# clovaai/frostnet

Hardware: AMD Instinct MI355X
Metric: images/sec FrostNet-Large 224x224 QAT fwd+bwd (higher is better)
Workload: dtype int8; 1 GPU; FrostNet-Large int8 fake-quant QAT fwd+bwd + GradBoost-SGD step (noise on; StatAssist FP epoch is a one-off before it), batch=512/GPU, 224x224 NHWC, qnnpack qconfig v0 (per-tensor); per_gpu_batch=512, global_batch=512, resolution=224, parallelism=dp1, hip_graph=True, grad_dtype=bf16

## Files before the change

frostnet_amd/_lib.py:

```python
import ctypes as C
import os

import torch

_HERE = os.path.dirname(os.path.abspath(__file__))
LIB_PATH = os.environ.get("FROST_HIP_LIB", os.path.join(_HERE, "libfrost_hip.so"))
_lib = None

P, I, L, F, D = C.c_void_p, C.c_int, C.c_int64, C.c_float, C.c_double

Q_MIN, Q_MAX, Q_SCALE, Q_ZP, Q_FQMIN, Q_FQMAX, Q_INV, Q_QMAX, Q_OBS_EN, Q_FQ_EN, Q_STRIDE = 0, 1, 2, 3, 4, 5, 6, 7, 8, 10, 12
COEF_ROWS = int(os.environ.get("FROST_COEF_ROWS_ALLOC", "14"))
COEF_ROWS_NAMED = 8
DWQ_NC, DWQ_SPREAD_MAX = int(os.environ.get("FROST_DWQ_NC", "4")), 32768
COEF_A, COEF_B = 0, 1
COEF_M, COEF_R, COEF_K1, COEF_S1, COEF_S2, COEF_VFRAC = 2, 3, 4, 5, 6, 7
STATS_BYTES_PER_CH = 24 * int(os.environ.get("FROST_STATS_TABLES", "4"))


class FrostWDesc(C.Structure):
    _fields_ = [("w", P), ("gamma", P), ("rvar", P), ("qrec", P), ("wq_pack", P), ("wsum", P), ("minmax2", P),
                ("wt_pack", P), ("wscale", P), ("wmin", P), ("wmax", P), ("cout", C.c_int32), ("cin_g", C.c_int32), ("kk", C.c_int32), ("kind", C.c_int32),
                ("cpad", C.c_int32), ("kpad", C.c_int32), ("reserved0", C.c_int32), ("reserved1", C.c_int32)]

# ... 125 lines not shown
    "frost_dw_conv_fwd_fin": [P, P, P, P, I, I, I, I, I, I, P, P, P],
    "frost_dw_conv_fwd": [P, P, P, P, I, I, I, I, I, I, I, P, P, P, I, P, P],
    "frost_stem_im2col": [P, P, I, I, I, P, P],
    "frost_stem_wgrad_remap": [P, I, I, P, P],
    "frost_conv_finalize": [P, L, I, P, P, P, P, P, P, P, I, I, I, P, P, P, P],
    "frost_cat_observe": [P, P, P, I, P],
    "frost_cat_requant": [P, P, I, P, P, I, L, P, P, P],
    "frost_add_minmax": [P, P, P, P, L, P, P],
    "frost_add_minmax_observe": [P, P, P, P, L, P, P, I, P],
    "frost_add_requant": [P, P, P, P, L, P, P, P],
    "frost_avgpool": [P, P, I, I, I, P, P, P],
    "frost_classifier_fwd": [P, P, P, P, I, I, I, P, P, P],
    "frost_pw_conv_bwd": [P, P, P, P, P, P, L, I, I, I, P, P, I, P, P, P, I, P],
    "frost_pw_wgrad": [P, P, P, L, I, I, P, P],
    "frost_pw_bwd_fused_ok": [L, I, I],
    "frost_pw_conv_int": [P, P, P, P, L, I, I, P, P],
    "frost_pw_ew": [P, L, I, P, P, I, I, P, P, P],
    "frost_pw_ew_emit_add": [P, L, I, P, P, I, P, P, P, P, P, I, P],
    "frost_pw_ew_add_bwd": [P, L, I, P, P, I, I, P, P, P, P, P, P, I, P, P],
    "frost_pw_conv_fwd_keep": [P, P, P, P, L, I, I, P, P, P, P],
    "frost_pwc_bwd_ok": [L, I, I],
    "frost_pwc_conv_bwd": [P, P, P, P, L, I, I, I, P, P, I, P, P, P],
    "frost_pwc_conv_fwd_emit": [P, P, P, P, L, I, I, P, P, P, P],
    "frost_block_supported": [I, I, I, I, I, I],
    "frost_block_fwd": [P, P],
    "frost_block_bwd": [P, P, P],
    "frost_block_expand_dw_stats": [P, P, P, P, P, P, P, I, I, I, I, I, P, P, I, P, P, P],
    "frost_block_dw_stats": [P, P, P, P, I, I, I, I, I, P, P, P],
    "frost_block_dw_reduce_supported": [I, I, I, I, I, I],
    "frost_block_dw_bwd_supported": [I, I, I, I, I],
    "frost_block_dw_bwd_reduce": [P, P, P, P, I, I, I, I, I, P, P, I, P, P],
    "frost_block_dw_bwd": [P, P, P, P, P, P, I, I, I, I, I, P, P, I, P, P, P, P],
    "frost_block_dw_bwd_c1": [P, P, P, P, P, P, I, I, I, I, I, P, P, I, P, P, P, P, P, P, P, P, I, I, P],
    "frost_block_dw_bwd_c1_ok": [I, I, I, I, I, I],
    "frost_block_dw_reduce": [P, P, P, P, P, P, I, P, I, I, I, I, I, P, P, I, P, P, P, P],
    "frost_pw_dgrad_wide_ok": [L, I, I],
    "frost_pw_dgrad_wide": [P, P, P, L, I, I, P, I, P],
    "frost_pw_conv_bwd_fused": [P, P, P, P, P, P, L, I, I, P, P, I, P, P, P, I, P, P],
    "frost_dw_conv_bwd": [P, P, P, P, P, I, I, I, I, I, I, I, P, P, I, P, P, P],
    "frost_dw_conv_bwd_dc_wgrad": [P, P, P, P, P, I, I, I, I, I, I, P, P, I, P, P, P, P],
    "frost_dw_dgrad": [P, P, P, I, I, I, I, I, I, P, I, P, P],
    "frost_dw_wgrad": [P, P, P, I, I, I, I, I, I, P, P],
    "frost_dw_bwd_fused_ok": [I, I, I, I, I],
    "frost_dw_bwd_fused": [P, P, P, P, P, P, I, I, I, I, I, I, P, P, I, P, P, P, P],
    "frost_dw_bwd_fused_c1_ok": [I, I, I, I, I, I],
    "frost_dw_bwd_fused_c1": [P, P, P, P, P, P, I, I, I, I, I, I, P, P, I, P, P, P, P, P, P, P, P, I, I, P],
# ... 196 lines not shown
```

frostnet_amd/csrc/frost_block.hip:

```cpp
#include "frost_common.h"

typedef int v2i __attribute__((ext_vector_type(2)));
#include <stdlib.h>

__device__ __forceinline__ int blk_xcd_item(int b, int total, int on) {
  if (!on || b >= (total & ~31)) return b;
  const int xcd = b & 7, j = b >> 3;
  return (j >> 2) * 32 + xcd * 4 + (j & 3);
}
__device__ __forceinline__ int blk_xcd_run(int b, int total, int run) {
  if (run < 2 || b >= total - total % (8 * run)) return b;
  const int xcd = b & 7, j = b >> 3;
  return (j / run) * (8 * run) + xcd * run + (j % run);
}
static int blk_xcd_on() { static const int on = getenv("FROST_BLK_XCD") ? atoi(getenv("FROST_BLK_XCD")) : 1; return on; }

struct BlkAP {
  const int8_t* x; const float* qx;
  const int8_t* w1; const int32_t* wsum1;
  const float* coef1; const float* qy1; int8_t* y1;
  const int8_t* wq2; const int32_t* wsum2;
  uint8_t* stats2; FrostFinDesc fin;
  int n, cin, c, cpad, KS, kstr, nchunk, csplit, imgs, rounds, xrun;
};
// ... 1459 lines not shown
  int cpw = cpw_env > 0 ? cpw_env : 2;
  if (cpw > p.nchunk) cpw = p.nchunk;
  p.csplit = (p.nchunk + cpw - 1) / cpw;
  static const int rounds_env = getenv("FROST_BLK_ROUNDS_A") ? atoi(getenv("FROST_BLK_ROUNDS_A")) : 0;
  p.imgs = imgs_env > 0 ? imgs_env : 0;
  p.rounds = rounds_env > 0 ? rounds_env : (h == 14 ? 2 : 1);
  hipStream_t s = as_stream(stream);
#define BLK_A(KK, HH, NWW, KSS) if (k == KK && h == HH && p.KS == KSS) return launch_blk_a<KK, HH, NWW, KSS>(p, s);
  BLK_A(3, 7, 4, 2) BLK_A(3, 7, 4, 3) BLK_A(3, 7, 4, 4) BLK_A(3, 7, 4, 5) BLK_A(5, 7, 4, 2) BLK_A(5, 7, 4, 3) BLK_A(5, 7, 4, 4) BLK_A(5, 7, 4, 5)
  BLK_A(3, 14, 8, 1) BLK_A(3, 14, 8, 2) BLK_A(3, 14, 8, 3) BLK_A(5, 14, 8, 1) BLK_A(5, 14, 8, 2) BLK_A(5, 14, 8, 3)
#undef BLK_A
  FROST_REQUIRE(false, "block_expand_dw: no instance");
  return 1;
}

extern "C" int frost_pw_conv_fwd_fin(const int8_t*, const float*, const int8_t*, const int32_t*, int64_t, int, int, void*, const FrostFinDesc*, void*);
extern "C" int frost_pw_ew(const int32_t*, int64_t, int, float*, const float*, int, int, const uint16_t*, void*, void*);
extern "C" int frost_pw_dgrad_wide(const uint16_t*, const uint16_t*, const float*, int64_t, int, int, uint16_t*, int, void*);
extern "C" int frost_pw_wgrad(const uint16_t*, const int8_t*, const float*, int64_t, int, int, float*, void*);
extern "C" int frost_pw_conv_bwd(const int8_t*, const float*, const int8_t*, const int32_t*, const uint16_t*, const float*, int64_t, int, int, int, float*, const float*, int,
                                 const uint16_t*, uint16_t*, uint16_t*, int, void*);
extern "C" int frost_pwc_bwd_ok(int64_t, int, int);
extern "C" int frost_pwc_conv_bwd(const int8_t*, const float*, const int8_t*, const int32_t*, int64_t, int, int, int, float*, const float*, int, const uint16_t*, uint16_t*, void*);

static int blk_desc_check(const FrostBlockDesc* d) {
  FROST_REQUIRE(d && d->x && d->y1 && d->y2 && d->y3 && d->conv_out3, "block: incomplete descriptor");
  FROST_REQUIRE(d->conv2.cout == d->conv1.cout && d->conv1.k == 1 && d->reduce.k == 1, "block: conv1 / reduce_conv are 1x1, conv2 is depthwise over conv1's channels");
  FROST_REQUIRE(frost_block_supported(d->h, d->w, d->conv2.k, 1, d->cin, d->conv1.cout) && frost_block_dw_reduce_supported(d->h, d->w, d->conv2.k, 1, d->conv1.cout, d->reduce.cout)
                && d->reduce.cout < d->conv1.cout, "block: unsupported shape (14x14 / 7x7 maps, depthwise stride 1, reduce_conv narrower than the expanded tensor)");
  return 0;
}

extern "C" int frost_block_fwd(const FrostBlockDesc* d, void* stream) {
  if (int rc = blk_desc_check(d)) return rc;
  const int64_t npix = (int64_t)d->n * d->h * d->w;
  const FrostBlockLayer &l1 = d->conv1, &l2 = d->conv2, &l3 = d->reduce;
  int rc = frost_pw_conv_fwd_fin(d->x, d->qrec_x, l1.wq_pack, l1.wsum, npix, d->cin, l1.cout, l1.stats, &l1.fin, stream);
  if (rc) return rc;
  rc = frost_block_expand_dw_stats(d->x, d->qrec_x, l1.wq_pack, l1.wsum, l1.fin.coef, l1.fin.qrec_y, d->y1, d->n, d->h, d->w, d->cin, l1.cout, l2.wq_pack, l2.wsum, l2.k, l2.stats,
                                   &l2.fin, stream);
  if (rc) return rc;
  rc = frost_block_dw_reduce(d->y1, l1.fin.qrec_y, l2.wq_pack, l2.wsum, l2.fin.coef, l2.fin.qrec_y, l2.fin.relu, d->y2, d->n, d->h, d->w, l1.cout, l2.k, l3.wq_pack, l3.wsum, l3.cout,
                             d->conv_out3, l3.stats, &l3.fin, stream);
  if (rc) return rc;
  return frost_pw_ew(d->conv_out3, npix, l3.cout, l3.fin.coef, l3.fin.qrec_y, l3.fin.relu, 2, nullptr, d->y3, stream);
}

extern "C" int frost_block_bwd(const FrostBlockDesc* d, const FrostBlockBwd* b, void* stream) {
  if (int rc = blk_desc_check(d)) return rc;
  FROST_REQUIRE(b && b->gout3 && b->dc3 && b->g2 && b->g1 && b->dc1, "block_bwd: incomplete gradient buffers");
  const int64_t npix = (int64_t)d->n * d->h * d->w;
  const FrostBlockLayer &l1 = d->conv1, &l2 = d->conv2, &l3 = d->reduce;
  hipStream_t ms = as_stream(stream), ss = b->side_stream ? as_stream(b->side_stream) : ms;
  hipEvent_t ev = nullptr;
  auto fork = [&]() { if (ss != ms) { if (!ev) hipEventCreateWithFlags(&ev, hipEventDisableTiming); hipEventRecord(ev, ms); hipStreamWaitEvent(ss, ev, 0); } };
  int rc;
  if ((rc = frost_pw_ew(d->conv_out3, npix, l3.cout, l3.fin.coef, l3.fin.qrec_y, l3.fin.relu, 0, b->gout3, nullptr, stream))) return rc;
  if ((rc = frost_pw_ew(d->conv_out3, npix, l3.cout, l3.fin.coef, l3.fin.qrec_y, l3.fin.relu, 1, b->gout3, b->dc3, stream))) return rc;
  fork();
  if ((rc = frost_pw_dgrad_wide(b->dc3, l3.wt_pack, l3.fin.qrec_w, npix, l1.cout, l3.cout, b->g2, 0, stream))) return rc;
  if ((rc = frost_pw_wgrad(b->dc3, d->y2, l2.fin.qrec_y, npix, l1.cout, l3.cout, l3.dwq, (void*)ss))) return rc;
  if ((rc = frost_block_dw_bwd_reduce(d->y1, l1.fin.qrec_y, l2.wq_pack, l2.wsum, d->n, d->h, d->w, l1.cout, l2.k, l2.fin.coef, l2.fin.qrec_y, l2.fin.relu, b->g2, stream))) return rc;
  if ((rc = frost_block_dw_bwd(d->y1, l1.fin.qrec_y, l2.wq_pack, l2.wsum, l2.fin.qrec_w, l2.fin.wscale, d->n, d->h, d->w, l1.cout, l2.k, l2.fin.coef, l2.fin.qrec_y, l2.fin.relu,
                               b->g2, b->g1, l2.dwq, stream))) return rc;
  const bool pwc = frost_pwc_bwd_ok(npix, d->cin, l1.cout) != 0;
  if (pwc && npix <= 131072) rc = frost_pwc_conv_bwd(d->x, d->qrec_x, l1.wq_pack, l1.wsum, npix, d->cin, l1.cout, 0, l1.fin.coef, l1.fin.qrec_y, l1.fin.relu, b->g1, nullptr, stream);
  else rc = frost_pw_conv_bwd(d->x, d->qrec_x, l1.wq_pack, l1.wsum, l1.wt_pack, l1.fin.qrec_w, npix, d->cin, l1.cout, 0, l1.fin.coef, l1.fin.qrec_y, l1.fin.relu, b->g1, nullptr, nullptr, 0, stream);
  if (rc) return rc;
  if (pwc) rc = frost_pwc_conv_bwd(d->x, d->qrec_x, l1.wq_pack, l1.wsum, npix, d->cin, l1.cout, 1, l1.fin.coef, l1.fin.qrec_y, l1.fin.relu, b->g1, b->dc1, stream);
  else rc = frost_pw_conv_bwd(d->x, d->qrec_x, l1.wq_pack, l1.wsum, l1.wt_pack, l1.fin.qrec_w, npix, d->cin, l1.cout, 1, l1.fin.coef, l1.fin.qrec_y, l1.fin.relu, b->g1, b->dc1, nullptr, 0, stream);
  if (rc) return rc;
  fork();
  if (b->dx && (rc = frost_pw_dgrad_wide(b->dc1, l1.wt_pack, l1.fin.qrec_w, npix, d->cin, l1.cout, b->dx, 0, stream))) return rc;
  if ((rc = frost_pw_wgrad(b->dc1, d->x, d->qrec_x, npix, d->cin, l1.cout, l1.dwq, (void*)ss))) return rc;
  if (ss != ms) {
    hipEventRecord(ev, ss); hipStreamWaitEvent(ms, ev, 0);
  }
  if (ev) hipEventDestroy(ev);
  return frost_check_launch("block_bwd");
}

struct SqCatP {
  const int8_t* x; const float* qx; const int8_t* w; const int32_t* wsum; const float* coef; const float* qsq; const float* qcat;
  int8_t* ysq; int8_t* ycat; int64_t npix; int cin, r, cpad, kstr;
  int cvt;
};
template <int KSM>
__global__ __launch_bounds__(256) void k_sq_emit_cat(const SqCatP p) {
  extern __shared__ __attribute__((aligned(16))) uint8_t smem[];
  uint8_t* const xs = smem;
  uint8_t* const lut = smem + 128 * p.kstr;
  const int tid = threadIdx.x, lane = tid & 63, wv = __builtin_amdgcn_readfirstlane(tid >> 6);
  const int j = lane & 15, g = lane >> 4;
  const int64_t p0 = (int64_t)blockIdx.x * 128;
  {
    const QP A = load_qp(p.qsq), B = load_qp(p.qx), Y = load_qp(p.qcat);
// ... 495 lines not shown
```

frostnet_amd/csrc/frost_pwc.hip:

```cpp
#include "frost_common.h"

struct PwcP {
  const int8_t* x; const float* qx; const int8_t* w; const int32_t* wsum;
  float* coef; const float* qy; const uint16_t* gout; uint16_t* dc; int8_t* y;
  int64_t npix; int cin, c, cpad, kstr, nchunk, csplit, relu, sr; float inv_count;
  uint8_t* stats; FrostFinDesc fin; unsigned fin_total; int ptpw; int64_t ntiles;
};

__device__ __forceinline__ void pwc_barrier() { asm volatile("s_waitcnt lgkmcnt(0)\n\ts_barrier" ::: "memory"); }
template <int CTRL>
__device__ __forceinline__ float pwc_dpp_add(float v) { return v + __int_as_float(__builtin_amdgcn_update_dpp(0, __float_as_int(v), CTRL, 0xf, 0xf, false)); }
__device__ __forceinline__ float pwc_row_sum(float v) { v = pwc_dpp_add<0x111>(v); v = pwc_dpp_add<0x112>(v); v = pwc_dpp_add<0x114>(v); v = pwc_dpp_add<0x118>(v); return v; }

#define PWC_PX 64
template <int MODE, int KSM>
__global__ __launch_bounds__(256, 4) void k_pwc(const PwcP p) {
  extern __shared__ __attribute__((aligned(16))) uint8_t smem[];
  uint8_t* const xs = smem;
  uint8_t* const gwin = smem + PWC_PX * p.kstr;
  const int tid = threadIdx.x, lane = tid & 63, w = __builtin_amdgcn_readfirstlane(tid >> 6);
  const int j = lane & 15, g = lane >> 4;
  const int cs = (int)blockIdx.x % p.csplit; const int64_t tile = (int64_t)blockIdx.x / p.csplit;
  const int chunk_lo = (cs * p.nchunk) / p.csplit, chunk_hi = ((cs + 1) * p.nchunk) / p.csplit;
  const int cw = (chunk_hi - chunk_lo) * 64;
// ... 179 lines not shown

extern "C" int frost_pwc_conv_bwd(const int8_t* x, const float* qrec_x, const int8_t* wq_pack, const int32_t* wsum, int64_t npix, int cin, int cout, int pass,
                                  float* coef, const float* qrec_y, int relu, const uint16_t* gout, uint16_t* dc, void* stream) {
  FROST_REQUIRE(frost_pwc_bwd_ok(npix, cin, cout) && (pass == 0 || (pass == 1 && dc)), "pwc_conv_bwd: unsupported layer or pass");
  PwcP p = {};
  p.x = x; p.qx = qrec_x; p.w = wq_pack; p.wsum = wsum; p.coef = coef; p.qy = qrec_y; p.gout = gout; p.dc = dc; p.npix = npix; p.cin = cin; p.c = cout;
  p.cpad = round_up(cout, 16); const int KS = (cin + 63) / 64; p.kstr = KS * 64 + 16; p.nchunk = (cout + 63) / 64; p.relu = relu; p.sr = frost_sr_enabled();
  p.inv_count = 1.0f / (float)npix;
  static const int cpw_env = getenv("FROST_PWC_CPW") ? atoi(getenv("FROST_PWC_CPW")) : 0;
  const int64_t tiles = (npix + PWC_PX - 1) / PWC_PX;
  int cpw = cpw_env > 0 ? cpw_env : (int)((tiles * p.nchunk + 2047) / 2048);
  if (cpw < 2) cpw = 2;
  if (cpw > p.nchunk) cpw = p.nchunk;
  if (cpw > 12) cpw = 12;
  p.csplit = (p.nchunk + cpw - 1) / cpw;
  hipStream_t s = as_stream(stream);
#define PWC_GO(KK) if (KS == KK) return pass == 0 ? launch_pwc<0, KK>(p, s) : launch_pwc<1, KK>(p, s);
  PWC_GO(1) PWC_GO(2) PWC_GO(3) PWC_GO(4) PWC_GO(5)
#undef PWC_GO
  FROST_REQUIRE(false, "pwc_conv_bwd: no instance");
  return 1;
}

extern "C" int frost_pwc_conv_fwd_emit(const int8_t* x, const float* qrec_x, const int8_t* wq_pack, const int32_t* wsum, int64_t npix, int cin, int cout,
                                       const float* coef, const float* qrec_y, int8_t* y, void* stream) {
  FROST_REQUIRE(frost_pwc_bwd_ok(npix, cin, cout) && y, "pwc_conv_fwd_emit: unsupported layer");
  PwcP p = {};
  p.x = x; p.qx = qrec_x; p.w = wq_pack; p.wsum = wsum; p.coef = (float*)coef; p.qy = qrec_y; p.y = y; p.npix = npix; p.cin = cin; p.c = cout;
  p.cpad = round_up(cout, 16); const int KS = (cin + 63) / 64; p.kstr = KS * 64 + 16; p.nchunk = (cout + 63) / 64;
  const int64_t tiles = (npix + PWC_PX - 1) / PWC_PX;
  int cpw = (int)((tiles * p.nchunk + 2047) / 2048);
  if (cpw < 2) cpw = 2;
  if (cpw > p.nchunk) cpw = p.nchunk;
  if (cpw > 12) cpw = 12;
  p.csplit = (p.nchunk + cpw - 1) / cpw;
  hipStream_t s = as_stream(stream);
#define PWC_GO(KK) if (KS == KK) return launch_pwc<2, KK>(p, s);
  PWC_GO(1) PWC_GO(2) PWC_GO(3) PWC_GO(4) PWC_GO(5)
#undef PWC_GO
  FROST_REQUIRE(false, "pwc_conv_fwd_emit: no instance");
  return 1;
}

template <int KSM>
__global__ __launch_bounds__(256, 4) void k_pwc_stats(const PwcP p) {
  extern __shared__ __attribute__((aligned(16))) uint8_t smem[];
// ... 130 lines not shown
```

frostnet_amd/engine.py:

```python
import ctypes as C
import os
from collections import namedtuple

import torch

from . import _lib as L
from ._lib import call, ptr, stream

SLACK = 256


def round_up(a, b):
    return (a + b - 1) // b * b


_DW_FUSE = os.environ.get("FROST_DW_FUSE", "1") != "0"
_PROLOGUE3 = os.environ.get("FROST_PROLOGUE3", "1") != "0"
_PROLOGUE3_CAP = int(os.environ.get("FROST_PROLOGUE3_CAP", "128"))
_DW_BWD_ONE = os.environ.get("FROST_DW_BWD_ONE", "1") != "0"
_DW_C1 = os.environ.get("FROST_DWB_C1", "3") != "0"
_PW_KEEP = os.environ.get("FROST_PW_KEEP", "1") != "0"
_FIN_FOLD = os.environ.get("FROST_FIN_FOLD", "1") != "0"
_BLOCK_FUSE = os.environ.get("FROST_BLOCK_FUSE", "1") != "0"
_BLOCK_PAIR = int(os.environ.get("FROST_BLOCK_PAIR", "3"))
# ... 171 lines not shown
            (self.rvar.data_ptr() if self.rvar is not None else None)
        d.qrec, d.wq_pack, d.wsum, d.minmax2 = self.qw.data_ptr(), self.wq_pack.data_ptr(), self.wsum.data_ptr(), \
            self.minmax2.data_ptr()
        d.wt_pack = self.wt_pack.data_ptr() if self.wt_pack is not None else None
        d.wscale = self.wscale.data_ptr()
        d.wmin, d.wmax = (self.wmin.data_ptr(), self.wmax.data_ptr()) if self.per_channel else (None, None)
        d.reserved1 = 1 if self.per_channel else 0
        d.cout, d.cin_g, d.kk, d.kind = self.cout, self.cin_g, self.kk, self.KIND_ID[self.kind]
        d.cpad, d.kpad = self.cpad, self.kpad
        d.reserved0 = 1 if self.fold_rsqrt else 0
        return d


class Engine:
    def __init__(self, device, rule127=False):
        self.device = torch.device(device)
        self.rule127 = 1 if rule127 else 0
        self.layers = []
        self.tape = []
        self._table = None
        self.on_layer_grads = None
        self._wgmap = None
        self._wg_stream, self._side, self._keep = None, None, []
        self.grad_fp32 = os.environ.get("FROST_GRAD", "bf16").lower() == "fp32"
        self.grad_mixed = os.environ.get("FROST_GRAD", "bf16").lower() == "mixed"
        self.mixed_max_hw = int(os.environ.get("FROST_GRAD_MIXED_HW", "14"))
        self.act_qmax = 255
        self.trace = None
        self._dbg, self._last_dc = False, None
        self.last_raw = self.last_logit_idx = None
        self._pending, self._frozen_stashed = [], []
        self._gtables = {}
        self._dwq_arena, self._dwq_layers = None, 0
        self._in_mm = self._add_mm = self._head_mm = self._hsw_present = self._sq_slots = self._g32_scratch = None
        self._prep_stream = None
        self._cfin_captured = self._cfin_warned = False

    def add_layer(self, layer):
        self.layers.append(layer)
        self._table = None
        return layer

    def _ensure_tables(self):
        if self._table is not None:
            return
        n = len(self.layers)
# ... 372 lines not shown
        call("frost_avgpool_q", ptr(x.buf), n, x.h * x.w, c, ptr(pooled), stream())
        self._finalize_converted(l, x.q, fb)
        logits = torch.empty(n, l.cout, dtype=torch.float32, device=self.device)
        self.last_logit_idx = torch.empty(n, l.cout, dtype=torch.uint8, device=self.device)
        call("frost_classifier_q_fb" if fb else "frost_classifier_q", ptr(pooled), ptr(x.q), ptr(l.wq_pack), ptr(l.coef), n, c, l.cout, ptr(l.qy), ptr(logits),
             ptr(self.last_logit_idx), stream())
        return logits

    def backward(self, dlogits=None, out_grads=None, boundaries=None, on_bucket=None):
        self._prepare_dwq()
        self._pending = []
        self._frozen_stashed = []
        try:
            if self.grad_fp32:
                return self._backward_g32(dlogits, boundaries, on_bucket)
            return self._backward_bf16(dlogits, boundaries, on_bucket)
        except BaseException:
            for l in self._frozen_stashed:
                self._frozen_restore(l)
            raise

    def _backward_bf16(self, dlogits, boundaries, on_bucket):
        self._side = None
        if _WG_STREAM and self.on_layer_grads is None and L.PROFILER is None and self.device.type == "cuda":
            if self._wg_stream is None:
                self._wg_stream = torch.cuda.Stream(device=self.device)
            self._side = self._wg_stream
            self._side.wait_stream(torch.cuda.current_stream())
            self._keep = []
        rtape = list(reversed(self.tape))
        for ti, node in enumerate(rtape):
            kind = node.kind
            if self.grad_mixed and self._mixed_entry(node):
                if kind == "conv":
                    self._layer_done(node.l, boundaries, on_bucket)
                continue
            if kind == "head":
                self._head_backward(node, dlogits)
                self._layer_done(node.l, boundaries, on_bucket)
            elif kind == "conv":
                self._conv_backward(node.l, node.x, node.y, producer_conv(rtape, ti, node.x))
                self._layer_done(node.l, boundaries, on_bucket)
            elif kind == "cat":
                a, b, y = node.a, node.b, node.y
                ga, fa = self._grad_slot(a)
                gb, fb = self._grad_slot(b)
                prod = producer_conv(rtape, ti, a)
                sq = prod.l if prod is not None and prod.x is b else None
                if _SQ_BWD_CAT and sq is not None and plain_pw(sq, per_tensor=True) and L.load_library().frost_sq_bwd_cat_ok(b.c, a.c):
                    call("frost_sq_bwd_cat", ptr(b.buf), ptr(b.q), ptr(sq.wq_pack), ptr(sq.wsum), b.npix, b.c, a.c, ptr(sq.coef), ptr(sq.qy), int(sq.relu), ptr(y.q),
                         ptr(y.grad), ptr(ga), fa, ptr(gb), fb, stream(), prof=("cat_bwd", 5 * y.numel + b.numel))
                    a.bred_done = True
                else:
                    call("frost_cat_bwd", ptr(y.grad), ptr(a.buf), ptr(a.q), a.c, ptr(b.buf), ptr(b.q), b.c, a.npix, ptr(y.q),
                         ptr(ga), fa, ptr(gb), fb, stream(), prof=("cat_bwd", 5 * y.numel))
# ... 140 lines not shown
        if self._dwq_arena is None or self._dwq_layers != len(self.layers):
            sizes = [self._dwq_elems(l.w.numel()) + (self._dwq_elems(l.cout * 40) if l.kind == "stem" else 0) for l in self.layers]
            self._dwq_arena = torch.empty(sum(sizes), dtype=torch.float32, device=self.device)
            o = 0
            for l, sz in zip(self.layers, sizes):
                l.dwq = self._dwq_arena[o: o + l.w.numel()]
                if l.kind == "stem":
                    o2 = o + self._dwq_elems(l.w.numel())
                    l.dwq_col = self._dwq_arena[o2: o2 + l.cout * 40]
                o += sz
            self._dwq_layers = len(self.layers)
            self._gtables = {}
        self._dwq_arena.zero_()

    def _fork_wgrad(self, *bufs):
        if self._side is None:
            return stream()
        ev = torch.cuda.Event()
        ev.record()
        self._side.wait_event(ev)
        self._keep.append(bufs)
        return C.c_void_p(self._side.cuda_stream)

    def _join_wgrad(self):
        if self._side is not None:
            torch.cuda.current_stream().wait_stream(self._side)
            self._keep = []

    def _close_bucket(self, index, on_bucket):
        self._join_wgrad()
        self._finalize_pending(slot=index)
        if on_bucket is not None:
            on_bucket(index)

    def _finalize_pending(self, slot=-1):
        if not self._pending:
            return
        for l in self._pending:
            self._ensure_grad(l)
        key = tuple((id(l), l.dwq.data_ptr(), l.w.grad.data_ptr(), l.gamma.grad.data_ptr(), l.beta.grad.data_ptr()) for l in self._pending)
        cache = self._gtables
        if slot not in cache or cache[slot][0] != key:
            arr = (L.FrostGDesc * len(self._pending))()
            for i, l in enumerate(self._pending):
                arr[i] = L.FrostGDesc(l.dwq.data_ptr(), l.w.data_ptr(), l.gamma.data_ptr(), l.sigma.data_ptr(), l.qw.data_ptr(),
                                      l.coef.data_ptr(), l.w.grad.data_ptr(), l.gamma.grad.data_ptr(), l.beta.grad.data_ptr(),
                                      l.cout, l.cin_g * l.kk, l.cpad, 0, l.wscale.data_ptr())
# ... 19 lines not shown
    def _dc_buffer(self, y, needed=True):
        dc = torch.empty(y.numel + 64, dtype=torch.int16, device=self.device) if needed else None
        if self._dbg:
            self._last_dc = dc
        return dc

    def _conv_backward(self, l, x, y, prod=None):
        self._ensure_grad(l)
        if l.kind == "dw":
            self._dw_backward(l, x, y, prod)
        elif l.kind in ("pw", "stem"):
            self._pw_backward(l, x, y)
        self._after_conv_backward(l, stream())
        y.grad = None

    def _pw_backward(self, l, x, y):
        gout = y.grad
        s = stream()
        fused = self._pw_fused(l, x)
        dc = self._dc_buffer(y, not fused)
        dwq = l.dwq_col if l.kind == "stem" else l.dwq
        args = (ptr(x.buf), ptr(x.q), ptr(l.wq_pack), ptr(l.wsum), ptr(l.wt_pack), ptr(l.qw), x.npix, x.c, l.cout)
        cint = None
        if keeps_conv_output(l, x) and not fused:
            cint = y.cint
            if cint is None:
                cint = torch.empty(y.numel + 64, dtype=torch.int32, device=self.device)
                call("frost_pw_conv_int", ptr(x.buf), ptr(x.q), ptr(l.wq_pack), ptr(l.wsum), x.npix, x.c, l.cout, ptr(cint), s,
                     prof=("pw_bwd_reduce", x.numel + 4 * y.numel))
            y.cint = None
            ab = y.add_bwd
            if ab is not None:
                call("frost_pw_ew_add_bwd", ptr(cint), x.npix, l.cout, ptr(l.coef), ptr(l.qy), int(l.relu), 0, ptr(ab[0]), ptr(ab[1].buf), ptr(ab[1].q), ptr(y.buf),
                     ptr(ab[2]), ptr(ab[3]), ab[4], None, s, prof=("pw_bwd_reduce", 10 * y.numel))
            else:
                call("frost_pw_ew", ptr(cint), x.npix, l.cout, ptr(l.coef), ptr(l.qy), int(l.relu), 0, ptr(gout), None, s,
                     prof=("pw_bwd_reduce", 6 * y.numel))
        else:
            pwc = (not fused) and l.kind == "pw" and bool(L.load_library().frost_pwc_bwd_ok(x.npix, x.c, l.cout))
            if y.bred_done:
                y.bred_done = False
            elif pwc and x.npix <= _PWC_RED_MAXPIX:
                call("frost_pwc_conv_bwd", ptr(x.buf), ptr(x.q), ptr(l.wq_pack), ptr(l.wsum), x.npix, x.c, l.cout, 0, ptr(l.coef), ptr(l.qy), int(l.relu), ptr(gout), None, s,
                     prof=("pw_bwd_reduce", x.numel + 2 * y.numel))
            else:
                call("frost_pw_conv_bwd", *args, 0, ptr(l.coef), ptr(l.qy), int(l.relu), ptr(gout), None, None, 0, s,
                     prof=("pw_bwd_reduce", x.numel + 2 * y.numel))
        self._frozen_after_reduce(l)
        if fused:
            gx, acc = self._grad_slot(x) if x.needs_grad else (None, 0)
            call("frost_pw_conv_bwd_fused", *args, ptr(l.coef), ptr(l.qy), int(l.relu), ptr(gout), ptr(dc), ptr(gx), acc, ptr(dwq), s,
                 prof=("pw_bwd_fused", x.numel + 2 * y.numel + (2 * x.numel if x.needs_grad else 0)))
            sw = s
        else:
            if cint is not None and y.add_bwd is not None:
                ab = y.add_bwd
                call("frost_pw_ew_add_bwd", ptr(cint), x.npix, l.cout, ptr(l.coef), ptr(l.qy), int(l.relu), 1, ptr(ab[0]), ptr(ab[1].buf), ptr(ab[1].q), ptr(y.buf),
                     ptr(ab[2]), None, 0, ptr(dc), s, prof=("pw_bwd_dc", 10 * y.numel))
                y.add_bwd = None
            elif cint is not None:
                call("frost_pw_ew", ptr(cint), x.npix, l.cout, ptr(l.coef), ptr(l.qy), int(l.relu), 1, ptr(gout), ptr(dc), s,
                     prof=("pw_bwd_dc", 8 * y.numel))
            elif pwc:
                call("frost_pwc_conv_bwd", ptr(x.buf), ptr(x.q), ptr(l.wq_pack), ptr(l.wsum), x.npix, x.c, l.cout, 1, ptr(l.coef), ptr(l.qy), int(l.relu), ptr(gout), ptr(dc), s,
                     prof=("pw_bwd_dc", x.numel + 4 * y.numel))
            else:
                call("frost_pw_conv_bwd", *args, 1, ptr(l.coef), ptr(l.qy), int(l.relu), ptr(gout), ptr(dc), None, 0, s,
                     prof=("pw_bwd_dc", x.numel + 4 * y.numel))
            sw = self._fork_wgrad(dc, x.buf)
            if x.needs_grad:
                gx, acc = self._grad_slot(x)
                if l.kind == "pw" and L.load_library().frost_pw_dgrad_wide_ok(x.npix, x.c, l.cout):
                    call("frost_pw_dgrad_wide", ptr(dc), ptr(l.wt_pack), ptr(l.qw), x.npix, x.c, l.cout, ptr(gx), acc, s,
                         prof=("pw_dgrad", 2 * y.numel + 2 * x.numel))
                else:
                    call("frost_pw_conv_bwd", *args, 2, ptr(l.coef), ptr(l.qy), int(l.relu), ptr(gout), ptr(dc), ptr(gx), acc, s,
                         prof=("pw_dgrad", 2 * y.numel + 2 * x.numel))
            call("frost_pw_wgrad", ptr(dc), ptr(x.buf), ptr(x.q), x.npix, x.c, l.cout, ptr(dwq), sw,
                 prof=("pw_wgrad", 2 * y.numel + x.numel))
        if l.kind == "stem":
            call("frost_stem_wgrad_remap", ptr(dwq), l.cout, l.cin_g, ptr(l.dwq), sw)

    def _dw_backward(self, l, x, y, prod):
        gout = y.grad
        s = stream()
        lib = L.load_library()
        blk = bool(_BLOCK_DWBWD and (x.h <= 7 or _BLOCK_DWBWD >= 2) and lib.frost_block_dw_bwd_supported(x.h, x.w, l.k, l.stride, x.c))
        fresh = x.grad is None
        if blk and (fresh or not x.needs_grad):
            path = "blk"
            fold = _BLOCK_C1 and x.needs_grad and conv1_foldable(prod, lib.frost_block_dw_bwd_c1_ok, (x.h, x.w, l.k, l.stride, x.c), k1=True)
        elif _DW_BWD_ONE and x.needs_grad and fresh and lib.frost_dw_bwd_fused_ok(x.h, x.w, x.c, l.k, l.stride):
            path = "one"
            fold = _DW_C1 and conv1_foldable(prod, lib.frost_dw_bwd_fused_c1_ok, (x.h, x.w, x.c, l.k, l.stride), k1=False)
        else:
            path, fold = "dc", False
        dc = self._dc_buffer(y, path == "dc")
        args = (ptr(x.buf), ptr(x.q), ptr(l.wq_pack), ptr(l.wsum), ptr(l.qw), x.n, x.h, x.w, x.c, l.k, l.stride)
        if blk and _BLOCK_DWBRED:
            call("frost_block_dw_bwd_reduce", ptr(x.buf), ptr(x.q), ptr(l.wq_pack), ptr(l.wsum), x.n, x.h, x.w, x.c, l.k, ptr(l.coef), ptr(l.qy), int(l.relu),
                 ptr(gout), s, prof=("blk_dw_bred", x.numel + 2 * y.numel))
        else:
# ... 79 lines not shown
```

include/frost_hip.h:

```cpp
#ifndef FROST_HIP_H
#define FROST_HIP_H
#include <stdint.h>

#ifdef __cplusplus
extern "C" {
#endif

#ifndef FROST_DWQ_NC
#define FROST_DWQ_NC 4
#endif
#define FROST_DWQ_SPREAD_MAX 32768
#define FROST_ABI_VERSION 5

#define FROST_Q_MIN 0
#define FROST_Q_MAX 1
#define FROST_Q_SCALE 2
#define FROST_Q_ZP 3
#define FROST_Q_FQMIN 4
#define FROST_Q_FQMAX 5
#define FROST_Q_INV 6
#define FROST_Q_QMAX 7
#define FROST_Q_OBS_EN 8
#define FROST_Q_FQ_EN 10
#define FROST_Q_STRIDE 12
// ... 320 lines not shown
  const float* cat_qrec_b; float* cat_qrec_y;
} FrostFinDesc;
int frost_pw_conv_fwd_fin(const int8_t* x, const float* qrec_x, const int8_t* wq_pack, const int32_t* wsum, int64_t npix, int cin, int cout,
                          void* stats, const FrostFinDesc* fin, void* stream);
int frost_sq_fwd_ok(int64_t npix, int cin, int r);
int64_t frost_sq_fwd_slot_bytes(int64_t npix, int r);
int frost_sq_fwd(const int8_t* x, const float* qrec_x, const int8_t* wq_pack, const int32_t* wsum, int64_t npix, int cin, int r, void* stats, const FrostFinDesc* fin,
                 void* slots, int8_t* y_sq, int8_t* y_cat, void* stream);
int frost_dw_conv_fwd_fin(const int8_t* x, const float* qrec_x, const int8_t* wq_pack, const int32_t* wsum, int n, int h, int w, int c, int k,
                          int stride, void* stats, const FrostFinDesc* fin, void* stream);
int frost_pw_conv_fwd_keep(const int8_t* x, const float* qrec_x, const int8_t* wq_pack, const int32_t* wsum, int64_t npix, int cin, int cout,
                           void* stats, const FrostFinDesc* fin, int32_t* conv_out, void* stream);

int frost_pw_ew_add_bwd(const int32_t* conv_out, int64_t npix, int cout, float* coef, const float* qrec_y, int relu, int mode, const uint16_t* gsum,
                        const int8_t* a, const float* qrec_a, const int8_t* yb, const float* qrec_sum, uint16_t* ga, int acc_a, uint16_t* dc, void* stream);
int frost_pw_ew_emit_add(const int32_t* conv_out, int64_t npix, int cout, const float* coef, const float* qrec_y, int relu, const int8_t* a,
                         const float* qrec_a, int8_t* y, float* state3, float* qrec_sum, int observe, void* stream);

int frost_pwc_bwd_ok(int64_t npix, int cin, int cout);
int frost_pwc_conv_fwd_emit(const int8_t* x, const float* qrec_x, const int8_t* wq_pack, const int32_t* wsum, int64_t npix, int cin, int cout,
                            const float* coef, const float* qrec_y, int8_t* y, void* stream);
int frost_pwc_conv_bwd(const int8_t* x, const float* qrec_x, const int8_t* wq_pack, const int32_t* wsum, int64_t npix, int cin, int cout, int pass,
                       float* coef, const float* qrec_y, int relu, const uint16_t* gout, uint16_t* dc, void* stream);

int frost_block_supported(int h, int w, int k, int stride, int cin, int c);
int frost_block_dw_stats(const int8_t* x, const float* qrec_x, const int8_t* wq_pack, const int32_t* wsum, int n, int h, int w, int c, int k, void* stats,
                         const FrostFinDesc* fin, void* stream);
int frost_block_expand_dw_stats(const int8_t* x, const float* qrec_x, const int8_t* w1_pack, const int32_t* wsum1, const float* coef1,
                                const float* qrec_y1, int8_t* y1, int n, int h, int w, int cin, int c, const int8_t* wq2, const int32_t* wsum2,
                                int k, void* stats2, const FrostFinDesc* fin2, void* stream);

int frost_block_dw_reduce_supported(int h, int w, int k, int stride, int c, int cout);
int frost_block_dw_reduce(const int8_t* y1, const float* qrec_y1, const int8_t* wq2, const int32_t* wsum2, const float* coef2, const float* qrec_y2,
                          int relu2, int8_t* y2, int n, int h, int w, int c, int k, const int8_t* w3_pack, const int32_t* wsum3, int cout,
                          int32_t* conv_out, void* stats3, const FrostFinDesc* fin3, void* stream);

int frost_block_dw_bwd_supported(int h, int w, int k, int stride, int c);
int frost_block_dw_bwd_reduce(const int8_t* x, const float* qrec_x, const int8_t* wq_pack, const int32_t* wsum, int n, int h, int w, int c, int k,
                              float* coef, const float* qrec_y, int relu, const uint16_t* gout, void* stream);
int frost_block_dw_bwd(const int8_t* x, const float* qrec_x, const int8_t* wq_pack, const int32_t* wsum, const float* qrec_w, const float* wscale,
                       int n, int h, int w, int c, int k, const float* coef, const float* qrec_y, int relu, const uint16_t* gout, uint16_t* dx,
                       float* dwq, void* stream);
int frost_block_dw_bwd_c1_ok(int h, int w, int k, int stride, int c, int c1_cin);
int frost_block_dw_bwd_c1(const int8_t* x, const float* qrec_x, const int8_t* wq_pack, const int32_t* wsum, const float* qrec_w, const float* wscale,
                          int n, int h, int w, int c, int k, const float* coef, const float* qrec_y, int relu, const uint16_t* gout, uint16_t* dx,
                          float* dwq, const int8_t* c1_x, const float* c1_qrec_x, const int8_t* c1_wq_pack, const int32_t* c1_wsum, float* c1_coef, int c1_cin,
// ... 191 lines not shown
```

Baseline: 26760 images/sec.

## Fuse pointwise conv backward dc computation with dgrad into one kernel

Adds a HIP kernel that recomputes the int8 pointwise conv output, forms the bf16 pre-activation gradient dc per tile, writes it out, and immediately multiplies it by the transposed weights to produce dx, all while the tile sits in LDS. This removes the separate dgrad_wide launch and its re-read of dc from global memory for eligible layers, in both the block path and the engine path. The engine also defers the weight-gradient launch for these layers by one tape step so it overlaps with later work on the side stream. In exchange, LDS use per block rises (up to 160 KB), which can lower occupancy, and the kernel adds register pressure from holding both accumulators.

```diff
diff --git a/frostnet_amd/_lib.py b/frostnet_amd/_lib.py
--- a/frostnet_amd/_lib.py
+++ b/frostnet_amd/_lib.py
@@ -171,6 +171,8 @@
     "frost_pwc_bwd_ok": [L, I, I],
     "frost_pwc_conv_bwd": [P, P, P, P, L, I, I, I, P, P, I, P, P, P],
     "frost_pwc_conv_fwd_emit": [P, P, P, P, L, I, I, P, P, P, P],
+    "frost_pwc_bwd_dcdx_ok": [L, I, I],
+    "frost_pwc_conv_bwd_dcdx": [P, P, P, P, P, P, L, I, I, P, P, I, P, P, P, I, P],
     "frost_block_supported": [I, I, I, I, I, I],
     "frost_block_fwd": [P, P],
     "frost_block_bwd": [P, P, P],
diff --git a/frostnet_amd/csrc/frost_block.hip b/frostnet_amd/csrc/frost_block.hip
--- a/frostnet_amd/csrc/frost_block.hip
+++ b/frostnet_amd/csrc/frost_block.hip
@@ -1505,6 +1505,9 @@
                                  const uint16_t*, uint16_t*, uint16_t*, int, void*);
 extern "C" int frost_pwc_bwd_ok(int64_t, int, int);
 extern "C" int frost_pwc_conv_bwd(const int8_t*, const float*, const int8_t*, const int32_t*, int64_t, int, int, int, float*, const float*, int, const uint16_t*, uint16_t*, void*);
+extern "C" int frost_pwc_bwd_dcdx_ok(int64_t, int, int);
+extern "C" int frost_pwc_conv_bwd_dcdx(const int8_t*, const float*, const int8_t*, const int32_t*, const uint16_t*, const float*, int64_t, int, int, float*, const float*, int,
+                                       const uint16_t*, uint16_t*, uint16_t*, int, void*);
 
 static int blk_desc_check(const FrostBlockDesc* d) {
   FROST_REQUIRE(d && d->x && d->y1 && d->y2 && d->y3 && d->conv_out3, "block: incomplete descriptor");
@@ -1550,11 +1553,14 @@
   if (pwc && npix <= 131072) rc = frost_pwc_conv_bwd(d->x, d->qrec_x, l1.wq_pack, l1.wsum, npix, d->cin, l1.cout, 0, l1.fin.coef, l1.fin.qrec_y, l1.fin.relu, b->g1, nullptr, stream);
   else rc = frost_pw_conv_bwd(d->x, d->qrec_x, l1.wq_pack, l1.wsum, l1.wt_pack, l1.fin.qrec_w, npix, d->cin, l1.cout, 0, l1.fin.coef, l1.fin.qrec_y, l1.fin.relu, b->g1, nullptr, nullptr, 0, stream);
   if (rc) return rc;
-  if (pwc) rc = frost_pwc_conv_bwd(d->x, d->qrec_x, l1.wq_pack, l1.wsum, npix, d->cin, l1.cout, 1, l1.fin.coef, l1.fin.qrec_y, l1.fin.relu, b->g1, b->dc1, stream);
+  const bool dcdx = pwc && b->dx && frost_pwc_bwd_dcdx_ok(npix, d->cin, l1.cout) != 0;
+  if (dcdx) rc = frost_pwc_conv_bwd_dcdx(d->x, d->qrec_x, l1.wq_pack, l1.wsum, l1.wt_pack, l1.fin.qrec_w, npix, d->cin, l1.cout, l1.fin.coef, l1.fin.qrec_y, l1.fin.relu, b->g1, b->dc1,
+                                         b->dx, 0, stream);
+  else if (pwc) rc = frost_pwc_conv_bwd(d->x, d->qrec_x, l1.wq_pack, l1.wsum, npix, d->cin, l1.cout, 1, l1.fin.coef, l1.fin.qrec_y, l1.fin.relu, b->g1, b->dc1, stream);
   else rc = frost_pw_conv_bwd(d->x, d->qrec_x, l1.wq_pack, l1.wsum, l1.wt_pack, l1.fin.qrec_w, npix, d->cin, l1.cout, 1, l1.fin.coef, l1.fin.qrec_y, l1.fin.relu, b->g1, b->dc1, nullptr, 0, stream);
   if (rc) return rc;
   fork();
-  if (b->dx && (rc = frost_pw_dgrad_wide(b->dc1, l1.wt_pack, l1.fin.qrec_w, npix, d->cin, l1.cout, b->dx, 0, stream))) return rc;
+  if (b->dx && !dcdx && (rc = frost_pw_dgrad_wide(b->dc1, l1.wt_pack, l1.fin.qrec_w, npix, d->cin, l1.cout, b->dx, 0, stream))) return rc;
   if ((rc = frost_pw_wgrad(b->dc1, d->x, d->qrec_x, npix, d->cin, l1.cout, l1.dwq, (void*)ss))) return rc;
   if (ss != ms) {
     hipEventRecord(ev, ss); hipStreamWaitEvent(ms, ev, 0);
diff --git a/frostnet_amd/csrc/frost_pwc.hip b/frostnet_amd/csrc/frost_pwc.hip
--- a/frostnet_amd/csrc/frost_pwc.hip
+++ b/frostnet_amd/csrc/frost_pwc.hip
@@ -225,6 +225,238 @@
   return 1;
 }
 
+typedef __bf16 pwc_v8bf16 __attribute__((ext_vector_type(8)));
+struct PwcDxP { PwcP p; const uint16_t* wt; const float* qw; uint16_t* dx; int accumulate, KB, CIT; };
+__device__ __forceinline__ int pwc_swz(int row, int part) { return part ^ ((row >> 1) & 7); }
+
+template <int KSM>
+__global__ __launch_bounds__(256, (KSM == 1 ? 4 : (KSM == 2 ? 3 : 2))) void k_pwc_dcdx(const PwcDxP q) {
+  const PwcP& p = q.p;
+  extern __shared__ __attribute__((aligned(16))) uint8_t smem[];
+  uint8_t* const xs = smem;
+  uint8_t* const gwin = smem + PWC_PX * p.kstr;
+  const int tid = threadIdx.x, lane = tid & 63, w = __builtin_amdgcn_readfirstlane(tid >> 6);
+  const int j = lane & 15, g = lane >> 4;
+  const int cw = p.nchunk * 64;
+  float* const tA = (float*)(gwin + 2 * PWC_PX * 64 * 2); float* const tB = tA + cw; float* const tK1 = tB + cw; float* const tE = tK1 + cw; float* const tF = tE + cw;
+  int* const tW = (int*)(tF + cw);
+  const int64_t p0 = (int64_t)blockIdx.x * PWC_PX;
+  const int CT = p.cpad >> 4;
+  for (int i = tid; i < cw; i += 256) {
+    const bool ok = i < p.c;
+    const int cc = ok ? i : 0;
+    float A = p.coef[FROST_COEF_A * p.cpad + cc], B = p.coef[FROST_COEF_B * p.cpad + cc], M = p.coef[FROST_COEF_M * p.cpad + cc], R = p.coef[FROST_COEF_R * p.cpad + cc];
+    int ws = p.wsum[cc];
+    float K1 = p.coef[FROST_COEF_K1 * p.cpad + cc], s1 = s12_sum(p.coef, p.cpad, 0, cc), s2 = s12_sum(p.coef, p.cpad, 1, cc);
+    if (!ok) { A = 0.0f; B = 0.0f; M = 0.0f; R = 0.0f; ws = 0; K1 = 0.0f; s1 = 0.0f; s2 = 0.0f; }
+    const float E = -K1 * (s2 * p.inv_count) * R;
+    tA[i] = A; tB[i] = B; tW[i] = ws; tK1[i] = K1; tE[i] = E; tF[i] = -K1 * (s1 * p.inv_count) - E * M;
+  }
+  {
+    const int upr = p.cin >> 3; const int64_t rows = p.npix - p0 < PWC_PX ? p.npix - p0 : PWC_PX; const int total = (int)rows * upr;
+    constexpr int XB = (PWC_PX * KSM * 8 + 255) / 256;
+    const int8_t* src = p.x + p0 * p.cin;
+    uint2 xv[XB];
+#pragma unroll
+    for (int i = 0; i < XB; ++i) { const int u = tid + i * 256; xv[i] = (u < total) ? *(const uint2*)(src + (int64_t)u * 8) : make_uint2(0, 0); }
+#pragma unroll
+    for (int i = 0; i < XB; ++i) {
+      const int u = tid + i * 256; const int row = u / upr, col = u - row * upr;
+      if (u < PWC_PX * upr) *(uint2*)(xs + row * p.kstr + col * 8) = xv[i];
+    }
+  }
+  const int zpx = __float_as_int(p.qx[FROST_Q_ZP]) - 128;
+  const float y_inv = 1.0f / p.qy[FROST_Q_SCALE];
+  float t_lo = 0.0f, t_hi;
+  {
+    const int zpy = __float_as_int(p.qy[FROST_Q_ZP]), qhi = q_hi(p.qy);
+    const float hi0 = (float)qhi + 0.5f - (float)zpy;
+    t_hi = ((qhi - zpy) & 1) ? __int_as_float(__float_as_int(hi0) - 1) : hi0;
+    if (!p.relu) { const float lo0 = -(float)zpy - 0.5f; t_lo = (zpy & 1) ? lo0 : __int_as_float(__float_as_int(lo0) + 1); }
+  }
+  uint32_t rng = sr_seed(blockIdx.x, threadIdx.x);
+  const int part = tid & 7, upx0 = tid >> 3, upx1 = (tid + 256) >> 3;
+  const bool pv0 = (p0 + upx0) < p.npix, pv1 = (p0 + upx1) < p.npix;
+  const int wo0 = upx0 * 128 + pwc_swz(upx0, part) * 16, wo1 = upx1 * 128 + pwc_swz(upx1, part) * 16;
+  auto load_g = [&](int chunk, uint4 (&dst)[2]) __attribute__((always_inline)) {
+    const bool cok = (chunk * 64 + part * 8) < p.c;
+    const uint16_t* gs = p.gout + p0 * p.c + chunk * 64 + part * 8;
+    dst[0] = (pv0 && cok) ? *(const uint4*)(gs + (int64_t)upx0 * p.c) : make_uint4(0, 0, 0, 0);
+    dst[1] = (pv1 && cok) ? *(const uint4*)(gs + (int64_t)upx1 * p.c) : make_uint4(0, 0, 0, 0);
+  };
+  auto load_w = [&](int chunk, v4i (&dst)[KSM]) __attribute__((always_inline)) {
+    const int ct = min(chunk * 4 + w, CT - 1);
+#pragma unroll
+    for (int ks = 0; ks < KSM; ++ks) dst[ks] = *(const v4i*)(p.w + ((((int64_t)ct * KSM + ks) * 64 + lane) << 4));
+  };
+  auto load_t = [&](int chunk, v4i (&dst)[KSM][2]) __attribute__((always_inline)) {
+#pragma unroll
+    for (int i = 0; i < KSM; ++i) {
+      const int ct = min(w + 4 * i, q.CIT - 1);
+#pragma unroll
+      for (int s = 0; s < 2; ++s) {
+        const int kb = min(chunk * 2 + s, q.KB - 1);
+        dst[i][s] = *(const v4i*)(q.wt + ((((int64_t)ct * q.KB + kb) * 64 + lane) << 3));
+      }
+    }
+  };
+  v4f dacc[KSM][4];
+#pragma unroll
+  for (int i = 0; i < KSM; ++i)
+#pragma unroll
+    for (int t = 0; t < 4; ++t) dacc[i][t] = (v4f){0.f, 0.f, 0.f, 0.f};
+  uint4 gv[2]; v4i afr[KSM]; v4i tfr[KSM][2];
+  load_g(0, gv); load_w(0, afr); load_t(0, tfr);
+  __syncthreads();
+
+  for (int chunk = 0; chunk < p.nchunk; ++chunk) {
+    uint8_t* const gw = gwin + (chunk & 1) * (PWC_PX * 64 * 2);
+    *(uint4*)(gw + wo0) = gv[0];
+    *(uint4*)(gw + wo1) = gv[1];
+    const int ti = chunk * 64 + w * 16 + 4 * g;
+    v4i acc[4];
+    {
+      const int4 ws = *(const int4*)(tW + ti); const v4i init = (v4i){-zpx * ws.x, -zpx * ws.y, -zpx * ws.z, -zpx * ws.w};
+#pragma unroll
+      for (int t = 0; t < 4; ++t) acc[t] = init;
+    }
+#pragma unroll
+    for (int ks = 0; ks < KSM; ++ks)
+#pragma unroll
+      for (int t = 0; t < 4; ++t) {
+        const v4i bfr = *(const v4i*)(xs + (t * 16 + j) * p.kstr + ks * 64 + g * 16);
+        acc[t] = __builtin_amdgcn_mfma_i32_16x16x64_i8(afr[ks], bfr, acc[t], 0, 0, 0);
+      }
+    if (chunk + 1 < p.nchunk) { load_g(chunk + 1, gv); load_w(chunk + 1, afr); }
+    pwc_barrier();
+    {
+      const float4 A4 = *(const float4*)(tA + ti), B4 = *(const float4*)(tB + ti);
+      const float A[4] = {A4.x, A4.y, A4.z, A4.w}, B[4] = {B4.x, B4.y, B4.z, B4.w};
+      const float4 K4 = *(const float4*)(tK1 + ti), E4 = *(const float4*)(tE + ti), F4 = *(const float4*)(tF + ti);
+      const float K1[4] = {K4.x, K4.y, K4.z, K4.w}, E[4] = {E4.x, E4.y, E4.z, E4.w}, F[4] = {F4.x, F4.y, F4.z, F4.w};
+#pragma unroll
+      for (int t = 0; t < 4; ++t) {
+        const int row = t * 16 + j;
+        uint8_t* const gp = gw + row * 128 + pwc_swz(row, 2 * w + (g >> 1)) * 16 + (g & 1) * 8;
+        const uint2 gq2 = *(const uint2*)gp;
+        const float gq[4] = {__uint_as_float(gq2.x << 16), __uint_as_float(gq2.x & 0xffff0000u), __uint_as_float(gq2.y << 16), __uint_as_float(gq2.y & 0xffff0000u)};
+        float dcv[4];
+#pragma unroll
+        for (int r = 0; r < 4; ++r) {
+          const float af = (float)acc[t][r];
+          const float tq = fmaf(A[r], af, B[r]) * y_inv;
+          const float gy = (tq > t_lo && tq <= t_hi) ? gq[r] : 0.0f;
+          dcv[r] = fmaf(gy, K1[r], fmaf(af, E[r], F[r]));
+        }
+        uint2 o;
+        if (p.sr) { o.x = sr_pk_bf16(dcv[0], dcv[1], rng); o.y = sr_pk_bf16(dcv[2], dcv[3], rng); }
+        else { o.x = cvt_pk_bf16(dcv[0], dcv[1]); o.y = cvt_pk_bf16(dcv[2], dcv[3]); }
+        *(uint2*)gp = o;
+      }
+    }
+    pwc_barrier();
+    {
+      const bool cok = (chunk * 64 + part * 8) < p.c;
+      uint16_t* dd = p.dc + p0 * p.c + chunk * 64 + part * 8;
+      if (pv0 && cok) *(uint4*)(dd + (int64_t)upx0 * p.c) = *(const uint4*)(gw + wo0);
+      if (pv1 && cok) *(uint4*)(dd + (int64_t)upx1 * p.c) = *(const uint4*)(gw + wo1);
+    }
+#pragma unroll
+    for (int s = 0; s < 2; ++s) {
+      if (chunk * 2 + s < q.KB) {
+#pragma unroll
+        for (int t = 0; t < 4; ++t) {
+          const int row = t * 16 + j;
+          const v4i b = *(const v4i*)(gw + row * 128 + pwc_swz(row, 4 * s + g) * 16);
+#pragma unroll
+          for (int i = 0; i < KSM; ++i)
+            if (w + 4 * i < q.CIT)
+              dacc[i][t] = __builtin_amdgcn_mfma_f32_16x16x32_bf16(__builtin_bit_cast(pwc_v8bf16, tfr[i][s]), __builtin_bit_cast(pwc_v8bf16, b), dacc[i][t], 0, 0, 0);
+        }
+      }
+    }
+    if (chunk + 1 < p.nchunk) load_t(chunk + 1, tfr);
+  }
+
+  const float sw = q.qw[FROST_Q_SCALE];
+  uint2 prev[KSM][4];
+  if (q.accumulate) {
+#pragma unroll
+    for (int i = 0; i < KSM; ++i) {
+      const int ci = (w + 4 * i) * 16 + 4 * g;
+#pragma unroll
+      for (int t = 0; t < 4; ++t) {
+        const int64_t px = p0 + 16 * t + j;
+        const bool ok = ci < p.cin && px < p.npix;
+        const uint2 o = *(const uint2*)(q.dx + (ok ? px * p.cin + ci : 0));
+        prev[i][t] = ok ? o : make_uint2(0u, 0u);
+      }
+    }
+  }
+  __syncthreads();
+  const int OP = p.cin * 2 + 16;
+#pragma unroll
+  for (int i = 0; i < KSM; ++i) {
+    if (w + 4 * i >= q.CIT) continue;
+    const int ci = (w + 4 * i) * 16 + 4 * g;
+#pragma unroll
+    for (int t = 0; t < 4; ++t) {
+      float v[4] = {dacc[i][t][0] * sw, dacc[i][t][1] * sw, dacc[i][t][2] * sw, dacc[i][t][3] * sw};
+      if (q.accumulate) { const uint2 o = prev[i][t]; v[0] += bf2f(o.x & 0xffff); v[1] += bf2f(o.x >> 16); v[2] += bf2f(o.y & 0xffff); v[3] += bf2f(o.y >> 16); }
+      uint2 o; o.x = cvt_pk_bf16(v[0], v[1]); o.y = cvt_pk_bf16(v[2], v[3]);
+      *(uint2*)(smem + (16 * t + j) * OP + ci * 2) = o;
+    }
+  }
+  __syncthreads();
+  {
+    const int upr = p.cin >> 3; const int64_t rows = p.npix - p0 < PWC_PX ? p.npix - p0 : PWC_PX; const int total = (int)rows * upr;
+    uint16_t* dst = q.dx + p0 * p.cin;
+    for (int u = tid; u < total; u += 256) {
+      const int row = u / upr, col = u - row * upr;
+      *(uint4*)(dst + (int64_t)u * 8) = *(const uint4*)(smem + row * OP + col * 16);
+    }
+  }
+}
+
+static size_t pwc_dcdx_lds(int cin, int cout) {
+  const int KS = (cin + 63) / 64, kstr = KS * 64 + 16, cw = ((cout + 63) / 64) * 64;
+  const size_t loop = (size_t)PWC_PX * kstr + 2 * PWC_PX * 64 * 2 + (size_t)cw * 4 * 6, out = (size_t)PWC_PX * (cin * 2 + 16);
+  return (loop > out ? loop : out) + 64;
+}
+extern "C" int frost_pwc_bwd_dcdx_ok(int64_t npix, int cin, int cout) {
+  static const int on = getenv("FROST_PWC_DCDX") ? atoi(getenv("FROST_PWC_DCDX")) : 1;
+  return (on && frost_pwc_bwd_ok(npix, cin, cout) && pwc_dcdx_lds(cin, cout) <= 160 * 1024) ? 1 : 0;
+}
+
+template <int KSM>
+static int launch_pwc_dcdx(PwcDxP& q, size_t lds, hipStream_t s) {
+  static bool attr_set = false;
+  if (lds > 64 * 1024 && !attr_set) { hipFuncSetAttribute((const void*)k_pwc_dcdx<KSM>, hipFuncAttributeMaxDynamicSharedMemorySize, 160 * 1024); attr_set = true; }
+  const int64_t tiles = (q.p.npix + PWC_PX - 1) / PWC_PX;
+  hipLaunchKernelGGL((k_pwc_dcdx<KSM>), dim3((unsigned)tiles), dim3(256), lds, s, q);
+  return frost_check_launch("pwc_dcdx");
+}
+
+extern "C" int frost_pwc_conv_bwd_dcdx(const int8_t* x, const float* qrec_x, const int8_t* wq_pack, const int32_t* wsum, const uint16_t* wt_pack, const float* qrec_w,
+                                       int64_t npix, int cin, int cout, float* coef, const float* qrec_y, int relu, const uint16_t* gout, uint16_t* dc,
+                                       uint16_t* dx, int accumulate, void* stream) {
+  FROST_REQUIRE(frost_pwc_bwd_dcdx_ok(npix, cin, cout) && dc && dx && wt_pack && qrec_w, "pwc_conv_bwd_dcdx: unsupported layer or missing buffer");
+  PwcDxP q = {};
+  PwcP& p = q.p;
+  p.x = x; p.qx = qrec_x; p.w = wq_pack; p.wsum = wsum; p.coef = coef; p.qy = qrec_y; p.gout = gout; p.dc = dc; p.npix = npix; p.cin = cin; p.c = cout;
+  p.cpad = round_up(cout, 16); const int KS = (cin + 63) / 64; p.kstr = KS * 64 + 16; p.nchunk = (cout + 63) / 64; p.csplit = 1; p.relu = relu; p.sr = frost_sr_enabled();
+  p.inv_count = 1.0f / (float)npix;
+  q.wt = wt_pack; q.qw = qrec_w; q.dx = dx; q.accumulate = accumulate;
+  q.KB = p.cpad / 32 + ((p.cpad % 32) ? 1 : 0); q.CIT = round_up(cin, 16) / 16;
+  const size_t lds = pwc_dcdx_lds(cin, cout);
+  hipStream_t s = as_stream(stream);
+#define PWC_GO(KK) if (KS == KK) return launch_pwc_dcdx<KK>(q, lds, s);
+  PWC_GO(1) PWC_GO(2) PWC_GO(3) PWC_GO(4) PWC_GO(5)
+#undef PWC_GO
+  FROST_REQUIRE(false, "pwc_conv_bwd_dcdx: no instance");
+  return 1;
+}
+
 extern "C" int frost_pwc_conv_fwd_emit(const int8_t* x, const float* qrec_x, const int8_t* wq_pack, const int32_t* wsum, int64_t npix, int cin, int cout,
                                        const float* coef, const float* qrec_y, int8_t* y, void* stream) {
   FROST_REQUIRE(frost_pwc_bwd_ok(npix, cin, cout) && y, "pwc_conv_fwd_emit: unsupported layer");
diff --git a/frostnet_amd/engine.py b/frostnet_amd/engine.py
--- a/frostnet_amd/engine.py
+++ b/frostnet_amd/engine.py
@@ -217,6 +217,7 @@
         self.on_layer_grads = None
         self._wgmap = None
         self._wg_stream, self._side, self._keep = None, None, []
+        self._late, self._late_prev = [], []
         self.grad_fp32 = os.environ.get("FROST_GRAD", "bf16").lower() == "fp32"
         self.grad_mixed = os.environ.get("FROST_GRAD", "bf16").lower() == "mixed"
         self.mixed_max_hw = int(os.environ.get("FROST_GRAD_MIXED_HW", "14"))
@@ -635,6 +636,7 @@
 
     def _backward_bf16(self, dlogits, boundaries, on_bucket):
         self._side = None
+        self._late, self._late_prev = [], []
         if _WG_STREAM and self.on_layer_grads is None and L.PROFILER is None and self.device.type == "cuda":
             if self._wg_stream is None:
                 self._wg_stream = torch.cuda.Stream(device=self.device)
@@ -644,6 +646,7 @@
         rtape = list(reversed(self.tape))
         for ti, node in enumerate(rtape):
             kind = node.kind
+            self._launch_late(False)
             if self.grad_mixed and self._mixed_entry(node):
                 if kind == "conv":
                     self._layer_done(node.l, boundaries, on_bucket)
@@ -830,7 +833,17 @@
         self._keep.append(bufs)
         return C.c_void_p(self._side.cuda_stream)
 
+    def _launch_late(self, every):
+        ready, self._late_prev = self._late_prev, []
+        if every:
+            ready, self._late = ready + self._late, []
+        else:
+            self._late_prev, self._late = self._late, []
+        for launch in ready:
+            launch()
+
     def _join_wgrad(self):
+        self._launch_late(True)
         if self._side is not None:
             torch.cuda.current_stream().wait_stream(self._side)
             self._keep = []
@@ -896,6 +909,7 @@
         dwq = l.dwq_col if l.kind == "stem" else l.dwq
         args = (ptr(x.buf), ptr(x.q), ptr(l.wq_pack), ptr(l.wsum), ptr(l.wt_pack), ptr(l.qw), x.npix, x.c, l.cout)
         cint = None
+        pwc = dcdx = False
         if keeps_conv_output(l, x) and not fused:
             cint = y.cint
             if cint is None:
@@ -912,6 +926,7 @@
                      prof=("pw_bwd_reduce", 6 * y.numel))
         else:
             pwc = (not fused) and l.kind == "pw" and bool(L.load_library().frost_pwc_bwd_ok(x.npix, x.c, l.cout))
+            dcdx = bool(pwc and x.needs_grad and L.load_library().frost_pwc_bwd_dcdx_ok(x.npix, x.c, l.cout))
             if y.bred_done:
                 y.bred_done = False
             elif pwc and x.npix <= _PWC_RED_MAXPIX:
@@ -935,6 +950,10 @@
             elif cint is not None:
                 call("frost_pw_ew", ptr(cint), x.npix, l.cout, ptr(l.coef), ptr(l.qy), int(l.relu), 1, ptr(gout), ptr(dc), s,
                      prof=("pw_bwd_dc", 8 * y.numel))
+            elif dcdx:
+                gx, acc = self._grad_slot(x)
+                call("frost_pwc_conv_bwd_dcdx", *args, ptr(l.coef), ptr(l.qy), int(l.relu), ptr(gout), ptr(dc), ptr(gx), acc, s,
+                     prof=("pw_bwd_dcdx", x.numel + 4 * y.numel + 2 * x.numel))
             elif pwc:
                 call("frost_pwc_conv_bwd", ptr(x.buf), ptr(x.q), ptr(l.wq_pack), ptr(l.wsum), x.npix, x.c, l.cout, 1, ptr(l.coef), ptr(l.qy), int(l.relu), ptr(gout), ptr(dc), s,
                      prof=("pw_bwd_dc", x.numel + 4 * y.numel))
@@ -942,7 +961,7 @@
                 call("frost_pw_conv_bwd", *args, 1, ptr(l.coef), ptr(l.qy), int(l.relu), ptr(gout), ptr(dc), None, 0, s,
                      prof=("pw_bwd_dc", x.numel + 4 * y.numel))
             sw = self._fork_wgrad(dc, x.buf)
-            if x.needs_grad:
+            if x.needs_grad and not dcdx:
                 gx, acc = self._grad_slot(x)
                 if l.kind == "pw" and L.load_library().frost_pw_dgrad_wide_ok(x.npix, x.c, l.cout):
                     call("frost_pw_dgrad_wide", ptr(dc), ptr(l.wt_pack), ptr(l.qw), x.npix, x.c, l.cout, ptr(gx), acc, s,
@@ -950,8 +969,12 @@
                 else:
                     call("frost_pw_conv_bwd", *args, 2, ptr(l.coef), ptr(l.qy), int(l.relu), ptr(gout), ptr(dc), ptr(gx), acc, s,
                          prof=("pw_dgrad", 2 * y.numel + 2 * x.numel))
-            call("frost_pw_wgrad", ptr(dc), ptr(x.buf), ptr(x.q), x.npix, x.c, l.cout, ptr(dwq), sw,
-                 prof=("pw_wgrad", 2 * y.numel + x.numel))
+            wgrad = lambda: call("frost_pw_wgrad", ptr(dc), ptr(x.buf), ptr(x.q), x.npix, x.c, l.cout, ptr(dwq), sw,
+                                 prof=("pw_wgrad", 2 * y.numel + x.numel))
+            if dcdx and self._side is not None:
+                self._late.append(wgrad)
+            else:
+                wgrad()
         if l.kind == "stem":
             call("frost_stem_wgrad_remap", ptr(dwq), l.cout, l.cin_g, ptr(l.dwq), sw)
 
diff --git a/include/frost_hip.h b/include/frost_hip.h
--- a/include/frost_hip.h
+++ b/include/frost_hip.h
@@ -366,6 +366,10 @@
                             const float* coef, const float* qrec_y, int8_t* y, void* stream);
 int frost_pwc_conv_bwd(const int8_t* x, const float* qrec_x, const int8_t* wq_pack, const int32_t* wsum, int64_t npix, int cin, int cout, int pass,
                        float* coef, const float* qrec_y, int relu, const uint16_t* gout, uint16_t* dc, void* stream);
+int frost_pwc_bwd_dcdx_ok(int64_t npix, int cin, int cout);
+int frost_pwc_conv_bwd_dcdx(const int8_t* x, const float* qrec_x, const int8_t* wq_pack, const int32_t* wsum, const uint16_t* wt_pack, const float* qrec_w,
+                            int64_t npix, int cin, int cout, float* coef, const float* qrec_y, int relu, const uint16_t* gout, uint16_t* dc,
+                            uint16_t* dx, int accumulate, void* stream);
 
 int frost_block_supported(int h, int w, int k, int stride, int cin, int c);
 int frost_block_dw_stats(const int8_t* x, const float* qrec_x, const int8_t* wq_pack, const int32_t* wsum, int n, int h, int w, int c, int k, void* stats,
```

Measured after the change: 26890 images/sec (median of 6 runs). About the same (+0.5%).
